# noamzilo/sed-crnn

Hardware: AMD Instinct MI355X
Metric: mel-frames/sec training throughput (seq=256, mel=40) (higher is better)
Workload: dtype f32; 1 GPU; BASELINE config 2: mono (B=128,256,40,1) per GPU, 3xConv3x3(128)+BN+ReLU+pool(1,2)+dropout0.5, BiGRU 2x128, Linear(256,1), BCEWithLogits, Adam lr 1e-3; full fit step (fwd+loss+bwd+allreduce+Adam); global_batch=128, seq_len=256, n_mels=40, parallelism=single

## Files before the change

### sed_crnn_amd/build.py

```python
import os
import subprocess
import sys
from concurrent.futures import ThreadPoolExecutor

HERE = os.path.dirname(os.path.abspath(__file__))
CSRC = os.path.join(HERE, "csrc")
OBJ = os.path.join(CSRC, "_obj")
LIB = os.path.join(HERE, "libsedcrnn.so")
SOURCES = ["api.cpp", "conv.hip", "conv_bf16.hip", "wino.hip", "conv1.hip", "bnpool.hip", "gemm.hip", "gru.hip", "misc.hip", "logmel.hip", "gcc.hip", "tdoa.hip", "doa.hip", "pcen.hip", "resample.hip", "data.hip", "detect.hip", "tune.hip", "stream.hip", "net.hip"]
FLAGS = ["--offload-arch=gfx950", "-O3", "-fPIC", "-std=c++17", "-Wall", "-Wno-unused-function"]
EXTRA_FLAGS = {"logmel.hip": ["-fno-slp-vectorize", "-Rpass-analysis=kernel-resource-usage"],
               "gcc.hip": ["-fno-slp-vectorize", "-Rpass-analysis=kernel-resource-usage"],
               "tdoa.hip": ["-fno-slp-vectorize", "-Rpass-analysis=kernel-resource-usage"],
               "doa.hip": ["-fno-slp-vectorize", "-Rpass-analysis=kernel-resource-usage"],
               "pcen.hip": ["-Rpass-analysis=kernel-resource-usage"],
               "conv.hip": ["-Rpass-analysis=kernel-resource-usage"],
               "wino.hip": ["-Rpass-analysis=kernel-resource-usage"],
               "conv_bf16.hip": ["-Rpass-analysis=kernel-resource-usage"]}
NO_SPILL_KERNELS = {"conv.hip": ("conv3x3_mfma_fwd2_k", "conv3x3_mfma_fwd_bf16x3_k")}
NO_SCRATCH_KERNELS = {"wino.hip": ("conv3x3_wino_k",),
                      "conv_bf16.hip": ("conv3x3_bf16_eval_k", "gemm_bf16_nt_k"),
                      "logmel.hip": ("logmel_fft_k",),
                      "gcc.hip": ("gcc_phat_k",),
                      "tdoa.hip": ("tdoa_accum_k", "tdoa_finish_k"),
                      "doa.hip": ("doa_steer_k",),
                      "pcen.hip": ("pcen_pass_k", "pcen_carry_k")}


def _hipcc():
    for c in (os.environ.get("HIPCC"), "/opt/rocm/bin/hipcc", "hipcc"):
        if c and (os.path.isabs(c) and os.path.exists(c) or not os.path.isabs(c)):
            return c
    raise RuntimeError("hipcc not found")


def _stale(target, deps):
    if not os.path.exists(target):
        return True
    t = os.path.getmtime(target)
    return any(os.path.getmtime(d) > t for d in deps)


def check_no_spill(remarks, kernels, allow_agprs=False):
    import re
    bad, seen, cur = [], set(), None
    for line in remarks.splitlines():
        m = re.search(r"remark: Function Name: (\S+)", line)
        if m:
            cur = next((k for k in kernels if k in m.group(1)), None)
            if cur:
                seen.add(cur)
            continue
        if cur:
            m = re.search(r"remark:\s+(ScratchSize \[bytes/lane\]|SGPRs Spill|VGPRs Spill|AGPRs): (\d+)", line)
            if m and int(m.group(2)) != 0 and not m.group(1).startswith("SGPRs") and not (allow_agprs and m.group(1) == "AGPRs"):
                bad.append(f"{cur}: {m.group(1)} = {m.group(2)}")
    bad += [f"{k}: no resource-usage remark found (kernel renamed? update NO_SPILL_KERNELS)" for k in kernels if k not in seen]
    return bad


def build(force=False, verbose=False):
    os.makedirs(OBJ, exist_ok=True)
    hipcc = _hipcc()
    headers = [os.path.join(CSRC, "common.h"), os.path.join(CSRC, "conv_shared.h"), os.path.join(CSRC, "detect_shared.h"), os.path.join(CSRC, "fft2048.h"), os.path.join(CSRC, "tdoa_shared.h"), os.path.join(HERE, "..", "include", "sedcrnn.h")]
    jobs = []
    objs = []
    for src in SOURCES:
        sp = os.path.join(CSRC, src)
        op = os.path.join(OBJ, os.path.splitext(src)[0] + ".o")
        objs.append(op)
        if force or _stale(op, [sp] + headers):
            cmd = [hipcc] + FLAGS + EXTRA_FLAGS.get(src, []) + (["-x", "hip"] if src.endswith(".cpp") else []) + ["-c", sp, "-o", op]
            jobs.append(cmd)

    def run(cmd):
        if verbose:
            print(" ".join(cmd), flush=True)
        r = subprocess.run(cmd, capture_output=True, text=True)
        if r.returncode != 0:
            raise RuntimeError("hipcc failed:\n" + " ".join(cmd) + "\n" + r.stdout + r.stderr)
        src = next((a for a in cmd if a.endswith((".hip", ".cpp"))), "")
        guarded = NO_SPILL_KERNELS.get(os.path.basename(src)) or NO_SCRATCH_KERNELS.get(os.path.basename(src))
        if guarded:
            bad = check_no_spill(r.stderr, guarded, allow_agprs=os.path.basename(src) in NO_SCRATCH_KERNELS)
            if bad:
                os.remove(cmd[cmd.index("-o") + 1])
                raise RuntimeError("hand-counted-waitcnt kernels must not spill:\n" + "\n".join(bad))
            keep, skip = [], 0
            for line in r.stderr.splitlines():
                if "remark:" in line:
                    skip = 2
                    continue
                if skip and (line.strip().startswith(("|", "^")) or " | " in line[:12]):
                    skip -= 1
                    continue
                skip = 0
                keep.append(line)
            return "\n".join(l for l in keep if l.strip() and "remarks generated" not in l)
        return r.stderr

    with ThreadPoolExecutor(max_workers=4) as ex:
        for warn in ex.map(run, jobs):
            if verbose and warn:
                print(warn)
    if force or jobs or _stale(LIB, objs):
        run([hipcc, "--offload-arch=gfx950", "-shared", "-fPIC", "-o", LIB] + objs)
    return LIB


if __name__ == "__main__":
    print(build(force="--force" in sys.argv, verbose=True))
```

### sed_crnn_amd/csrc/gru.hip

```cpp
#include "common.h"

static inline int gru_bt(int H, int B) {
    int bt = B >= 512 ? 4 : (B >= 256 ? 2 : 1);
    if (H >= 128 && bt > 2) bt = 2;
    return bt;
}

__global__ void gru_pack_whh_t_k(const float* __restrict__ w0, const float* __restrict__ w1,
                                 float* __restrict__ wt, int H) {
    int i = blockIdx.x * blockDim.x + threadIdx.x;
    int n = 3 * H * H;
    if (i >= 2 * n) return;
    int dir = i / n, e = i - dir * n;
    int g = e / H, k = e - g * H;
    const float* w = dir ? w1 : w0;
    wt[(size_t)dir * n + (size_t)k * 3 * H + g] = w[e];
}

constexpr int gru_nt(int hreg) { return hreg > 0 ? ((3 * hreg + 63) / 64) * 64 : 1024; }

__device__ __forceinline__ float gru_dot4(float w0, float w1, float w2, float w3, const f32x4& h) {
    return fmaf(w3, h[3], fmaf(w2, h[2], fmaf(w0, h[0], w1 * h[1])));
}

template <int HREG, int GRU_BT, int HTOT = HREG, int HLDS = 0>
__global__ __launch_bounds__(gru_nt(HTOT)) void gru_seq_fwd_k(
    const float* __restrict__ gi, const float* __restrict__ wt, const float* __restrict__ bhh0,
    const float* __restrict__ bhh1, float* __restrict__ out, float* __restrict__ saved, int B, int T, int H) {
    extern __shared__ __attribute__((aligned(16))) float smem[];
    float* h_s = smem;
    float* gh_s = smem + GRU_BT * H;
    float* w_l = smem + GRU_BT * 4 * H;
    const int g = threadIdx.x;
    const int dir = blockIdx.y, b0 = blockIdx.x * GRU_BT;
    const int H3 = 3 * H;
    const float* wtd = wt + (size_t)dir * H3 * H;
    const float* bhh = dir ? bhh1 : bhh0;
    const bool row = g < H3;
    const bool gate = g < H;
    constexpr bool HYB = HTOT != HREG && HREG > 0;

    float wreg[HREG > 0 ? HREG : 1];
    if (HREG > 0 && row) {
#pragma unroll
        for (int k = 0; k < HREG; ++k) wreg[k] = wtd[(size_t)k * H3 + g];
    }
    if (HYB && row) {
        for (int j = 0; j < HLDS; ++j) w_l[j * H3 + g] = wtd[(size_t)(HREG + j) * H3 + g];
    }
    const float bias = row ? bhh[g] : 0.f;
    for (int i = g; i < GRU_BT * H; i += blockDim.x) h_s[i] = 0.f;
    __syncthreads();

    float gr[GRU_BT], gz[GRU_BT], gn[GRU_BT], nr[GRU_BT], nz[GRU_BT], nn[GRU_BT], mr[GRU_BT], mz[GRU_BT], mn[GRU_BT];
    auto fetch_gi = [&](int s, float* a, float* bq, float* c) {
        const int tt = dir ? (T - 1 - s) : s;
#pragma unroll
        for (int b = 0; b < GRU_BT; ++b) {
            int bg = b0 + b;
            if (gate && bg < B && s < T) {
                const float* p = gi + (((size_t)bg * T + tt) * 2 + dir) * H3;
                a[b] = p[g]; bq[b] = p[H + g]; c[b] = p[2 * H + g];
            } else { a[b] = bq[b] = c[b] = 0.f; }
        }
    };
    fetch_gi(0, gr, gz, gn);
    fetch_gi(1, nr, nz, nn);
    for (int s = 0; s < T; ++s) {
        const int tt = dir ? (T - 1 - s) : s;
        fetch_gi(s + 2, mr, mz, mn);
        if (row) {
            float acc[GRU_BT];
#pragma unroll
            for (int b = 0; b < GRU_BT; ++b) acc[b] = bias;
            if (HREG > 0) {
#pragma unroll
                for (int k = 0; k < HREG; k += 4) {
#pragma unroll
                    for (int b = 0; b < GRU_BT; ++b) {
                        f32x4 hv = *(const f32x4*)(h_s + b * H + k);
                        acc[b] += gru_dot4(wreg[k], wreg[k + 1], wreg[k + 2], wreg[k + 3], hv);
                    }
                }
            }
            if (HYB) {
#pragma unroll 4
                for (int j = 0; j < HLDS; j += 4) {
                    const float w0 = w_l[j * H3 + g], w1 = w_l[(j + 1) * H3 + g], w2 = w_l[(j + 2) * H3 + g], w3 = w_l[(j + 3) * H3 + g];
#pragma unroll
                    for (int b = 0; b < GRU_BT; ++b) {
                        f32x4 hv = *(const f32x4*)(h_s + b * H + HREG + j);
                        acc[b] += gru_dot4(w0, w1, w2, w3, hv);
                    }
                }
            }
            if (HREG == 0 || HYB) {
                for (int k = HYB ? HREG + HLDS : 0; k < H; k += 4) {
                    float w0 = wtd[(size_t)k * H3 + g], w1 = wtd[(size_t)(k + 1) * H3 + g];
                    float w2 = wtd[(size_t)(k + 2) * H3 + g], w3 = wtd[(size_t)(k + 3) * H3 + g];
#pragma unroll
                    for (int b = 0; b < GRU_BT; ++b) {
                        f32x4 hv = *(const f32x4*)(h_s + b * H + k);
                        acc[b] += gru_dot4(w0, w1, w2, w3, hv);
                    }
                }
            }
#pragma unroll
            for (int b = 0; b < GRU_BT; ++b) gh_s[b * H3 + g] = acc[b];
        }
        __syncthreads();
        if (gate) {
#pragma unroll
            for (int b = 0; b < GRU_BT; ++b) {
                int bg = b0 + b;
                float ghr = gh_s[b * H3 + g], ghz = gh_s[b * H3 + H + g], ghn = gh_s[b * H3 + 2 * H + g];
                float hp = h_s[b * H + g];
                float r = __fdividef(1.f, 1.f + __expf(-(gr[b] + ghr)));
                float z = __fdividef(1.f, 1.f + __expf(-(gz[b] + ghz)));
                float a = gn[b] + r * ghn;
                float e2 = __expf(-2.f * fabsf(a));
                float n = copysignf(__fdividef(1.f - e2, 1.f + e2), a);
                float hn = (1.f - z) * n + z * hp;
                h_s[b * H + g] = hn;
                if (bg < B) {
                    out[((size_t)bg * T + tt) * 2 * H + dir * H + g] = hn;
                    if (saved) {
                        float* sp = saved + ((((size_t)bg * T + tt) * 2 + dir) * 5) * H + g;
                        sp[0] = r; sp[H] = z; sp[2 * H] = n; sp[3 * H] = ghn; sp[4 * H] = hp;
                    }
                }
            }
        }
#pragma unroll
        for (int b = 0; b < GRU_BT; ++b) {
            gr[b] = nr[b]; gz[b] = nz[b]; gn[b] = nn[b];
            nr[b] = mr[b]; nz[b] = mz[b]; nn[b] = mn[b];
        }
        __syncthreads();
    }
}

template <int HREG, int GRU_BT, int HTOT = HREG, int HLDS = 0>
__global__ __launch_bounds__(gru_nt(HTOT)) void gru_seq_bwd_k(
    const float* __restrict__ dout, const float* __restrict__ saved, const float* __restrict__ whh0,
    const float* __restrict__ whh1, float* __restrict__ dgi, float* __restrict__ dgh, float* __restrict__ bpart,
    int B, int T, int H) {
    extern __shared__ __attribute__((aligned(16))) float smem[];
    const int H3 = 3 * H;
    float* dgh_s = smem;
    float* part_s = smem + GRU_BT * H3;
    float* w_l = smem + GRU_BT * 2 * H3;
    const int g = threadIdx.x;
    const int dir = blockIdx.y, b0 = blockIdx.x * GRU_BT;
    const float* whh = dir ? whh1 : whh0;
    const bool row = g < H3;
    const bool gate = g < H;
    const int p = g / H, k = g - p * H;
    constexpr bool HYB = HTOT != HREG && HREG > 0;

    float wreg[HREG > 0 ? HREG : 1];
    if (HREG > 0 && row) {
#pragma unroll
        for (int j = 0; j < HREG; ++j) wreg[j] = whh[((size_t)p * H + j) * H + k];
    }
    if (HYB && row) {
        for (int j = 0; j < HLDS; ++j) w_l[j * H3 + g] = whh[((size_t)p * H + HREG + j) * H + k];
    }
    for (int i = g; i < 3 * GRU_BT * H; i += blockDim.x) part_s[i] = 0.f;
    float dhc[GRU_BT];
#pragma unroll
    for (int b = 0; b < GRU_BT; ++b) dhc[b] = 0.f;
    float sb0 = 0.f, sb1 = 0.f, sb2 = 0.f, sb3 = 0.f;
    __syncthreads();

    float cs[GRU_BT][6], ns[GRU_BT][6], ms[GRU_BT][6];
    auto fetch_sv = [&](int s, float (*q)[6]) {
        const int tt = dir ? s : (T - 1 - s);
#pragma unroll
        for (int b = 0; b < GRU_BT; ++b) {
            int bg = b0 + b;
            if (gate && bg < B && s < T) {
                const float* sp = saved + ((((size_t)bg * T + tt) * 2 + dir) * 5) * H + g;
                q[b][0] = sp[0]; q[b][1] = sp[H]; q[b][2] = sp[2 * H]; q[b][3] = sp[3 * H]; q[b][4] = sp[4 * H];
                q[b][5] = dout[((size_t)bg * T + tt) * 2 * H + dir * H + g];
            }
        }
    };
    constexpr bool AHEAD2 = !(HREG == 0 && GRU_BT == 4) && !HYB;
    fetch_sv(0, cs);
    if (AHEAD2) fetch_sv(1, ns);
    for (int s = 0; s < T; ++s) {
        const int tt = dir ? s : (T - 1 - s);
        if (AHEAD2) fetch_sv(s + 2, ms);
        else fetch_sv(s + 1, ns);
        if (gate) {
#pragma unroll
            for (int b = 0; b < GRU_BT; ++b) {
                int bg = b0 + b;
                float dr_pre = 0.f, dz_pre = 0.f, dn_pre = 0.f, dghn = 0.f, carry = 0.f;
                if (bg < B) {
                    float r = cs[b][0], z = cs[b][1], n = cs[b][2], ghn = cs[b][3], hp = cs[b][4];
                    float dh = cs[b][5] + dhc[b] +
                               part_s[(0 * GRU_BT + b) * H + g] + part_s[(1 * GRU_BT + b) * H + g] +
                               part_s[(2 * GRU_BT + b) * H + g];
                    float dn = dh * (1.f - z);
                    float dz = dh * (hp - n);
                    carry = dh * z;
                    dn_pre = dn * (1.f - n * n);
                    dz_pre = dz * z * (1.f - z);
                    float dr = dn_pre * ghn;
                    dghn = dn_pre * r;
                    dr_pre = dr * r * (1.f - r);
                    size_t o = (((size_t)bg * T + tt) * 2 + dir) * H3 + g;
                    dgi[o] = dr_pre; dgi[o + H] = dz_pre; dgi[o + 2 * H] = dn_pre;
                    dgh[o] = dr_pre; dgh[o + H] = dz_pre; dgh[o + 2 * H] = dghn;
                }
                dhc[b] = carry;
                sb0 += dr_pre; sb1 += dz_pre; sb2 += dn_pre; sb3 += dghn;
                dgh_s[b * H3 + g] = dr_pre; dgh_s[b * H3 + H + g] = dz_pre; dgh_s[b * H3 + 2 * H + g] = dghn;
            }
        }
        __syncthreads();
        if (row) {
            float acc[GRU_BT];
#pragma unroll
            for (int b = 0; b < GRU_BT; ++b) acc[b] = 0.f;
            if (HREG > 0) {
#pragma unroll
                for (int j = 0; j < HREG; j += 4) {
#pragma unroll
                    for (int b = 0; b < GRU_BT; ++b) {
                        f32x4 dv = *(const f32x4*)(dgh_s + b * H3 + p * H + j);
                        acc[b] += wreg[j] * dv[0] + wreg[j + 1] * dv[1] + wreg[j + 2] * dv[2] + wreg[j + 3] * dv[3];
                    }
                }
            }
            if (HYB) {
#pragma unroll 4
                for (int j = 0; j < HLDS; j += 4) {
                    const float w0 = w_l[j * H3 + g], w1 = w_l[(j + 1) * H3 + g], w2 = w_l[(j + 2) * H3 + g], w3 = w_l[(j + 3) * H3 + g];
#pragma unroll
                    for (int b = 0; b < GRU_BT; ++b) {
                        f32x4 dv = *(const f32x4*)(dgh_s + b * H3 + p * H + HREG + j);
                        acc[b] += w0 * dv[0] + w1 * dv[1] + w2 * dv[2] + w3 * dv[3];
                    }
                }
            }
            if (HREG == 0 || HYB) {
                for (int j = HYB ? HREG + HLDS : 0; j < H; j += 4) {
                    const float* wp = whh + ((size_t)p * H + j) * H + k;
                    float w0 = wp[0], w1 = wp[H], w2 = wp[2 * H], w3 = wp[3 * H];
#pragma unroll
                    for (int b = 0; b < GRU_BT; ++b) {
                        f32x4 dv = *(const f32x4*)(dgh_s + b * H3 + p * H + j);
                        acc[b] += w0 * dv[0] + w1 * dv[1] + w2 * dv[2] + w3 * dv[3];
                    }
                }
            }
#pragma unroll
            for (int b = 0; b < GRU_BT; ++b) part_s[(p * GRU_BT + b) * H + k] = acc[b];
        }
#pragma unroll
        for (int b = 0; b < GRU_BT; ++b)
#pragma unroll
            for (int e = 0; e < 6; ++e) { cs[b][e] = ns[b][e]; if (AHEAD2) ns[b][e] = ms[b][e]; }
        __syncthreads();
    }
    if (bpart && gate) {
        float* bp = bpart + ((size_t)(blockIdx.x * 2 + dir) * 4) * H + g;
        bp[0] = sb0; bp[H] = sb1; bp[2 * H] = sb2; bp[3 * H] = sb3;
    }
}

__global__ void gru_bias_grad_k(const float* __restrict__ bpart, int nblk, int H, float* __restrict__ dbih0,
                                float* __restrict__ dbih1, float* __restrict__ dbhh0, float* __restrict__ dbhh1) {
    int i = blockIdx.x * blockDim.x + threadIdx.x;
    if (i >= 2 * 4 * H) return;
    int j = i % H, c = (i / H) % 4, dir = i / (4 * H);
    float a = 0.f;
#pragma unroll 8
    for (int b = 0; b < nblk; ++b) a += bpart[((size_t)(b * 2 + dir) * 4 + c) * H + j];
    float* dbih = dir ? dbih1 : dbih0;
    float* dbhh = dir ? dbhh1 : dbhh0;
    if (c < 3) dbih[c * H + j] = a;
    if (c < 2) dbhh[c * H + j] = a;
    if (c == 3) dbhh[2 * H + j] = a;
}

static int gru_threads(int H) { return ((3 * H + 63) / 64) * 64; }
#define GRU_HR 96
#define GRU_HL 48
#define GRU_HR_FWD 116

extern "C" size_t sed_gru_seq_workspace_bytes(int H) { return (size_t)2 * 3 * H * H * sizeof(float); }

struct GruVariant { int bt, hreg, hlds; };
static inline GruVariant gru_variant(int H, int B, int hyb_hreg) {
    const int bt = gru_bt(H, B);
    if (H == 8 || H == 16 || H == 32 || H == 64 || H == 128) return {bt, H, 0};
    if (H == 256 && bt == 1) return {bt, hyb_hreg, GRU_HL};
    return {bt, 0, 0};
}

extern "C" int sed_gru_seq_variant(int B, int H, int* bt, int* hreg, int* hlds) {
    SED_REQUIRE(bt && hreg && hlds, "gru_seq_variant: null pointer");
    SED_REQUIRE(B > 0 && H > 0 && H % 4 == 0 && 3 * H <= 1024, "gru_seq_variant: H=%d must be a multiple of 4 and <= 341", H);
    const GruVariant v = gru_variant(H, B, GRU_HR_FWD);
    *bt = v.bt; *hreg = v.hreg; *hlds = v.hlds;
    return 0;
}

#define GRU_BT3(HR, KERNEL, ...)                                                              \
    if (v.bt == 1) KERNEL<HR, 1><<<grid, nt, lds, s>>>(__VA_ARGS__);                          \
    else if (v.bt == 2) KERNEL<HR, 2><<<grid, nt, lds, s>>>(__VA_ARGS__);                     \
    else KERNEL<HR, 4><<<grid, nt, lds, s>>>(__VA_ARGS__)
#define GRU_DISPATCH(KERNEL, ...)                                                             \
    if (v.hlds > 0) {                                                                         \
        KERNEL<GRU_HRX, 1, 256, GRU_HL><<<grid, nt, lds + (size_t)GRU_HL * 768 * sizeof(float), s>>>(__VA_ARGS__); \
    } else switch (v.hreg) {                                                                  \
        case 8: GRU_BT3(8, KERNEL, __VA_ARGS__); break;                                       \
        case 16: GRU_BT3(16, KERNEL, __VA_ARGS__); break;                                     \
        case 32: GRU_BT3(32, KERNEL, __VA_ARGS__); break;                                     \
        case 64: GRU_BT3(64, KERNEL, __VA_ARGS__); break;                                     \
        case 128:                                                                             \
            if (v.bt == 1) KERNEL<128, 1><<<grid, nt, lds, s>>>(__VA_ARGS__);                 \
            else KERNEL<128, 2><<<grid, nt, lds, s>>>(__VA_ARGS__);                           \
            break;                                                                            \
        default: GRU_BT3(0, KERNEL, __VA_ARGS__); break;                                      \
    }

extern "C" int sed_gru_seq_fwd(const float* gi, const float* const* whh, const float* const* bhh, float* out,
                               float* saved, void* workspace, int B, int T, int H, void* stream) {
    SED_REQUIRE(gi && whh && bhh && out && workspace && whh[0] && whh[1] && bhh[0] && bhh[1], "gru_seq_fwd: null pointer");
    SED_REQUIRE(B > 0 && T > 0 && H > 0 && H % 4 == 0 && 3 * H <= 1024, "gru_seq_fwd: H=%d must be a multiple of 4 and <= 341", H);
    hipStream_t s = as_stream(stream);
    float* wt = (float*)workspace;
    int n = 2 * 3 * H * H;
    gru_pack_whh_t_k<<<cdiv(n, 256), 256, 0, s>>>(whh[0], whh[1], wt, H);
    SED_LAUNCH_CHECK("gru_pack_whh_t");
    const GruVariant v = gru_variant(H, B, GRU_HR_FWD);
    dim3 grid(cdiv(B, v.bt), 2);
    int nt = gru_threads(H);
    size_t lds = (size_t)v.bt * 4 * H * sizeof(float);
    SedProfScope prof(SED_K_GRU_FWD, s, 2.0 * 2 * B * (double)T * 3 * H * H);
    if (v.hlds > 0)
        (void)hipFuncSetAttribute((const void*)gru_seq_fwd_k<GRU_HR_FWD, 1, 256, GRU_HL>, hipFuncAttributeMaxDynamicSharedMemorySize, 160 * 1024);
#define GRU_HRX GRU_HR_FWD
    GRU_DISPATCH(gru_seq_fwd_k, gi, wt, bhh[0], bhh[1], out, saved, B, T, H);
#undef GRU_HRX
    SED_LAUNCH_CHECK("gru_seq_fwd");
    return 0;
}

extern "C" size_t sed_gru_seq_bwd_workspace_bytes(int B, int H) { return (size_t)cdiv(B, gru_bt(H, B)) * 2 * 4 * H * sizeof(float); }

extern "C" int sed_gru_seq_bwd(const float* dout, const float* saved, const float* const* whh, float* dgi,
                               float* dgh, float* const* dbih, float* const* dbhh, void* workspace, int B, int T,
                               int H, void* stream) {
    SED_REQUIRE(dout && saved && whh && whh[0] && whh[1] && dgi && dgh, "gru_seq_bwd: null pointer");
    const bool want_bias = dbih && dbhh;
    SED_REQUIRE(!want_bias || (workspace && dbih[0] && dbih[1] && dbhh[0] && dbhh[1]), "gru_seq_bwd: bias gradients need all four outputs and a workspace");
    float* bpart = want_bias ? (float*)workspace : nullptr;
    SED_REQUIRE(B > 0 && T > 0 && H > 0 && H % 4 == 0 && 3 * H <= 1024, "gru_seq_bwd: H=%d must be a multiple of 4 and <= 341", H);
    hipStream_t s = as_stream(stream);
    const GruVariant v = gru_variant(H, B, GRU_HR);
    dim3 grid(cdiv(B, v.bt), 2);
    int nt = gru_threads(H);
    size_t lds = (size_t)v.bt * 6 * H * sizeof(float);
    SedProfScope prof(SED_K_GRU_BWD, s, 2.0 * 2 * B * (double)T * 3 * H * H);
    if (v.hlds > 0)
        (void)hipFuncSetAttribute((const void*)gru_seq_bwd_k<GRU_HR, 1, 256, GRU_HL>, hipFuncAttributeMaxDynamicSharedMemorySize, 160 * 1024);
#define GRU_HRX GRU_HR
    GRU_DISPATCH(gru_seq_bwd_k, dout, saved, whh[0], whh[1], dgi, dgh, bpart, B, T, H);
#undef GRU_HRX
    SED_LAUNCH_CHECK("gru_seq_bwd");
    if (want_bias) {
        gru_bias_grad_k<<<cdiv(8 * H, 256), 256, 0, s>>>(bpart, cdiv(B, v.bt), H, dbih[0], dbih[1], dbhh[0], dbhh[1]);
        SED_LAUNCH_CHECK("gru_bias_grad");
    }
    return 0;
}
```

Measured before the change: 5.902 million mel-frames/s.

## Software-pipeline GRU recurrence with inline-asm loads and hand-counted vmcnt waits

Rewrites the forward and backward GRU sequence kernels to use a rotating three-slot prefetch buffer. Per-step gate inputs and saved activations are fetched with inline-asm global loads, and the code waits on explicit vmcnt counts instead of letting the compiler insert full waits. The register matvec is split into batched LDS loads with sched barriers, and the step loop is unrolled by three so buffer indices are compile-time constants. The build now guards these kernels against spills, because the hand-counted waits and register pinning break if the compiler spills. Out-of-range batch and time indices are clamped instead of masked.

```diff
diff --git a/sed_crnn_amd/build.py b/sed_crnn_amd/build.py
--- a/sed_crnn_amd/build.py
+++ b/sed_crnn_amd/build.py
@@ -16,8 +16,10 @@
                "pcen.hip": ["-Rpass-analysis=kernel-resource-usage"],
                "conv.hip": ["-Rpass-analysis=kernel-resource-usage"],
                "wino.hip": ["-Rpass-analysis=kernel-resource-usage"],
-               "conv_bf16.hip": ["-Rpass-analysis=kernel-resource-usage"]}
-NO_SPILL_KERNELS = {"conv.hip": ("conv3x3_mfma_fwd2_k", "conv3x3_mfma_fwd_bf16x3_k")}
+               "conv_bf16.hip": ["-Rpass-analysis=kernel-resource-usage"],
+               "gru.hip": ["-Rpass-analysis=kernel-resource-usage"]}
+NO_SPILL_KERNELS = {"conv.hip": ("conv3x3_mfma_fwd2_k", "conv3x3_mfma_fwd_bf16x3_k"),
+                    "gru.hip": ("gru_seq_fwd_k", "gru_seq_bwd_k")}
 NO_SCRATCH_KERNELS = {"wino.hip": ("conv3x3_wino_k",),
                       "conv_bf16.hip": ("conv3x3_bf16_eval_k", "gemm_bf16_nt_k"),
                       "logmel.hip": ("logmel_fft_k",),
diff --git a/sed_crnn_amd/csrc/gru.hip b/sed_crnn_amd/csrc/gru.hip
--- a/sed_crnn_amd/csrc/gru.hip
+++ b/sed_crnn_amd/csrc/gru.hip
@@ -21,6 +21,46 @@
 
 __device__ __forceinline__ float gru_dot4(float w0, float w1, float w2, float w3, const f32x4& h) {
     return fmaf(w3, h[3], fmaf(w2, h[2], fmaf(w0, h[0], w1 * h[1])));
+}
+
+template <int N> __device__ __forceinline__ void gru_vmcnt() {
+    static_assert(N >= 0 && N <= 63, "vmcnt is a 6-bit field on gfx9");
+    asm volatile("s_waitcnt vmcnt(%0)" ::"n"(N) : "memory");
+}
+__device__ __forceinline__ void gru_load(float& dst, unsigned voff, const float* sbase) {
+    asm volatile("global_load_dword %0, %1, %2" : "=&v"(dst) : "v"(voff), "s"(sbase) : "memory");
+}
+template <int V> struct GruC { static constexpr int value = V; };
+
+template <int HREG, int BT, int LB>
+__device__ __forceinline__ void gru_dot_reg(const float (&w)[HREG > 0 ? HREG : 1], const float* x, int stride, float (&acc)[BT]) {
+    constexpr int NQ = HREG / 4 * BT, NB = (NQ + LB - 1) / LB;
+    f32x4 v[2][LB];
+#pragma unroll
+    for (int j = 0; j < LB; ++j)
+        if (j < NQ) v[0][j] = *(const f32x4*)(x + (j % BT) * stride + (j / BT) * 4);
+    __builtin_amdgcn_sched_barrier(0);
+#pragma unroll
+    for (int nb = 0; nb < NB; ++nb) {
+#pragma unroll
+        for (int j = 0; j < LB; ++j) {
+            const int i = (nb + 1) * LB + j;
+            if (i < NQ) v[(nb + 1) & 1][j] = *(const f32x4*)(x + (i % BT) * stride + (i / BT) * 4);
+        }
+        const int last = (nb + 1) * LB <= NQ ? LB - 1 : NQ - nb * LB - 1;
+        __builtin_amdgcn_sched_barrier(0);
+        asm volatile("" : "+v"(v[nb & 1][last]));
+        __builtin_amdgcn_sched_barrier(0);
+#pragma unroll
+        for (int j = 0; j < LB; ++j) {
+            const int i = nb * LB + j;
+            if (i < NQ) {
+                const int k = (i / BT) * 4;
+                acc[i % BT] += gru_dot4(w[k], w[k + 1], w[k + 2], w[k + 3], v[nb & 1][j]);
+            }
+        }
+        __builtin_amdgcn_sched_barrier(0);
+    }
 }
 
 template <int HREG, int GRU_BT, int HTOT = HREG, int HLDS = 0>
@@ -39,6 +79,7 @@
     const bool row = g < H3;
     const bool gate = g < H;
     constexpr bool HYB = HTOT != HREG && HREG > 0;
+    constexpr bool ROT = !HYB;
 
     float wreg[HREG > 0 ? HREG : 1];
     if (HREG > 0 && row) {
@@ -52,28 +93,13 @@
     for (int i = g; i < GRU_BT * H; i += blockDim.x) h_s[i] = 0.f;
     __syncthreads();
 
-    float gr[GRU_BT], gz[GRU_BT], gn[GRU_BT], nr[GRU_BT], nz[GRU_BT], nn[GRU_BT], mr[GRU_BT], mz[GRU_BT], mn[GRU_BT];
-    auto fetch_gi = [&](int s, float* a, float* bq, float* c) {
-        const int tt = dir ? (T - 1 - s) : s;
-#pragma unroll
-        for (int b = 0; b < GRU_BT; ++b) {
-            int bg = b0 + b;
-            if (gate && bg < B && s < T) {
-                const float* p = gi + (((size_t)bg * T + tt) * 2 + dir) * H3;
-                a[b] = p[g]; bq[b] = p[H + g]; c[b] = p[2 * H + g];
-            } else { a[b] = bq[b] = c[b] = 0.f; }
-        }
-    };
-    fetch_gi(0, gr, gz, gn);
-    fetch_gi(1, nr, nz, nn);
-    for (int s = 0; s < T; ++s) {
-        const int tt = dir ? (T - 1 - s) : s;
-        fetch_gi(s + 2, mr, mz, mn);
+    auto matvec = [&](float b_hh) __attribute__((always_inline)) {
         if (row) {
             float acc[GRU_BT];
 #pragma unroll
-            for (int b = 0; b < GRU_BT; ++b) acc[b] = bias;
-            if (HREG > 0) {
+            for (int b = 0; b < GRU_BT; ++b) acc[b] = b_hh;
+            if (HREG > 0 && ROT) gru_dot_reg<HREG, GRU_BT, 8>(wreg, h_s, H, acc);
+            if (HREG > 0 && !ROT) {
 #pragma unroll
                 for (int k = 0; k < HREG; k += 4) {
 #pragma unroll
@@ -108,35 +134,112 @@
 #pragma unroll
             for (int b = 0; b < GRU_BT; ++b) gh_s[b * H3 + g] = acc[b];
         }
-        __syncthreads();
+    };
+    auto gates = [&](int tt, const float (&q)[GRU_BT][3], bool sv) __attribute__((always_inline)) {
         if (gate) {
 #pragma unroll
             for (int b = 0; b < GRU_BT; ++b) {
                 int bg = b0 + b;
                 float ghr = gh_s[b * H3 + g], ghz = gh_s[b * H3 + H + g], ghn = gh_s[b * H3 + 2 * H + g];
                 float hp = h_s[b * H + g];
-                float r = __fdividef(1.f, 1.f + __expf(-(gr[b] + ghr)));
-                float z = __fdividef(1.f, 1.f + __expf(-(gz[b] + ghz)));
-                float a = gn[b] + r * ghn;
+                float r = __fdividef(1.f, 1.f + __expf(-(q[b][0] + ghr)));
+                float z = __fdividef(1.f, 1.f + __expf(-(q[b][1] + ghz)));
+                float a = q[b][2] + r * ghn;
                 float e2 = __expf(-2.f * fabsf(a));
                 float n = copysignf(__fdividef(1.f - e2, 1.f + e2), a);
                 float hn = (1.f - z) * n + z * hp;
                 h_s[b * H + g] = hn;
-                if (bg < B) {
+                if (GRU_BT == 1 || bg < B) {
                     out[((size_t)bg * T + tt) * 2 * H + dir * H + g] = hn;
-                    if (saved) {
+                    if (sv) {
                         float* sp = saved + ((((size_t)bg * T + tt) * 2 + dir) * 5) * H + g;
                         sp[0] = r; sp[H] = z; sp[2 * H] = n; sp[3 * H] = ghn; sp[4 * H] = hp;
                     }
                 }
             }
         }
-#pragma unroll
-        for (int b = 0; b < GRU_BT; ++b) {
-            gr[b] = nr[b]; gz[b] = nz[b]; gn[b] = nn[b];
-            nr[b] = mr[b]; nz[b] = mz[b]; nn[b] = mn[b];
-        }
-        __syncthreads();
+    };
+
+    constexpr int AHEAD = 2, NSET = AHEAD + 1;
+    float pf[NSET][GRU_BT][3];
+    if constexpr (ROT) {
+        const int gq = g % H;
+        const unsigned vo0 = 4u * gq, vo1 = 4u * (H + gq), vo2 = 4u * (2 * H + gq);
+        auto fetch_gi = [&](int s, float (&q)[GRU_BT][3]) __attribute__((always_inline)) {
+            const int sc = s < T ? s : T - 1;
+            const int tt = dir ? (T - 1 - sc) : sc;
+#pragma unroll
+            for (int b = 0; b < GRU_BT; ++b) {
+                const int bg = b0 + b < B ? b0 + b : B - 1;
+                const float* p = gi + (((size_t)bg * T + tt) * 2 + dir) * H3;
+                gru_load(q[b][0], vo0, p); gru_load(q[b][1], vo1, p); gru_load(q[b][2], vo2, p);
+            }
+        };
+        fetch_gi(0, pf[0]);
+        fetch_gi(1, pf[1]);
+        gru_vmcnt<0>();
+        if (HREG > 0) {
+#pragma unroll
+            for (int k = 0; k < HREG; ++k) asm volatile("" : "+v"(wreg[k]));
+        }
+        float bias_r = bias;
+        asm volatile("" : "+v"(bias_r));
+
+        auto step = [&](int s, auto RC, auto SV) __attribute__((always_inline)) {
+            constexpr int R = decltype(RC)::value;
+            constexpr bool SAVED = decltype(SV)::value != 0;
+            constexpr int NWAIT = AHEAD * 3 * GRU_BT + (GRU_BT == 1 ? AHEAD * (SAVED ? 6 : 1) : 0);
+            fetch_gi(s + AHEAD, pf[(R + AHEAD) % NSET]);
+            matvec(bias_r);
+            __syncthreads();
+            gru_vmcnt<NWAIT>();
+#pragma unroll
+            for (int b = 0; b < GRU_BT; ++b)
+#pragma unroll
+                for (int e = 0; e < 3; ++e) asm volatile("" : "+v"(pf[R][b][e]));
+            gates(dir ? (T - 1 - s) : s, pf[R], SAVED);
+            __syncthreads();
+        };
+        auto run = [&](auto SV) __attribute__((always_inline)) {
+            int s = 0;
+            for (; s + NSET <= T; s += NSET) { step(s, GruC<0>{}, SV); step(s + 1, GruC<1>{}, SV); step(s + 2, GruC<2>{}, SV); }
+            if (s < T) step(s, GruC<0>{}, SV);
+            if (s + 1 < T) step(s + 1, GruC<1>{}, SV);
+        };
+        if (saved) run(GruC<1>{});
+        else run(GruC<0>{});
+        gru_vmcnt<0>();
+#pragma unroll
+        for (int r = 0; r < NSET; ++r)
+#pragma unroll
+            for (int b = 0; b < GRU_BT; ++b)
+#pragma unroll
+                for (int e = 0; e < 3; ++e) asm volatile("" : "+v"(pf[r][b][e]));
+    } else {
+        auto fetch_gi = [&](int s, float (&q)[GRU_BT][3]) __attribute__((always_inline)) {
+            const int tt = dir ? (T - 1 - s) : s;
+#pragma unroll
+            for (int b = 0; b < GRU_BT; ++b) {
+                int bg = b0 + b;
+                if (gate && bg < B && s < T) {
+                    const float* p = gi + (((size_t)bg * T + tt) * 2 + dir) * H3;
+                    q[b][0] = p[g]; q[b][1] = p[H + g]; q[b][2] = p[2 * H + g];
+                } else { q[b][0] = q[b][1] = q[b][2] = 0.f; }
+            }
+        };
+        fetch_gi(0, pf[0]);
+        fetch_gi(1, pf[1]);
+        for (int s = 0; s < T; ++s) {
+            fetch_gi(s + 2, pf[2]);
+            matvec(bias);
+            __syncthreads();
+            gates(dir ? (T - 1 - s) : s, pf[0], saved != nullptr);
+#pragma unroll
+            for (int b = 0; b < GRU_BT; ++b)
+#pragma unroll
+                for (int e = 0; e < 3; ++e) { pf[0][b][e] = pf[1][b][e]; pf[1][b][e] = pf[2][b][e]; }
+            __syncthreads();
+        }
     }
 }
 
@@ -157,6 +260,7 @@
     const bool gate = g < H;
     const int p = g / H, k = g - p * H;
     constexpr bool HYB = HTOT != HREG && HREG > 0;
+    constexpr bool ROT = HREG == HTOT && HREG > 0 && HREG * GRU_BT < 256;
 
     float wreg[HREG > 0 ? HREG : 1];
     if (HREG > 0 && row) {
@@ -173,32 +277,13 @@
     float sb0 = 0.f, sb1 = 0.f, sb2 = 0.f, sb3 = 0.f;
     __syncthreads();
 
-    float cs[GRU_BT][6], ns[GRU_BT][6], ms[GRU_BT][6];
-    auto fetch_sv = [&](int s, float (*q)[6]) {
-        const int tt = dir ? s : (T - 1 - s);
-#pragma unroll
-        for (int b = 0; b < GRU_BT; ++b) {
-            int bg = b0 + b;
-            if (gate && bg < B && s < T) {
-                const float* sp = saved + ((((size_t)bg * T + tt) * 2 + dir) * 5) * H + g;
-                q[b][0] = sp[0]; q[b][1] = sp[H]; q[b][2] = sp[2 * H]; q[b][3] = sp[3 * H]; q[b][4] = sp[4 * H];
-                q[b][5] = dout[((size_t)bg * T + tt) * 2 * H + dir * H + g];
-            }
-        }
-    };
-    constexpr bool AHEAD2 = !(HREG == 0 && GRU_BT == 4) && !HYB;
-    fetch_sv(0, cs);
-    if (AHEAD2) fetch_sv(1, ns);
-    for (int s = 0; s < T; ++s) {
-        const int tt = dir ? s : (T - 1 - s);
-        if (AHEAD2) fetch_sv(s + 2, ms);
-        else fetch_sv(s + 1, ns);
+    auto gates = [&](int tt, const float (&cs)[GRU_BT][6]) __attribute__((always_inline)) {
         if (gate) {
 #pragma unroll
             for (int b = 0; b < GRU_BT; ++b) {
                 int bg = b0 + b;
                 float dr_pre = 0.f, dz_pre = 0.f, dn_pre = 0.f, dghn = 0.f, carry = 0.f;
-                if (bg < B) {
+                if (GRU_BT == 1 || bg < B) {
                     float r = cs[b][0], z = cs[b][1], n = cs[b][2], ghn = cs[b][3], hp = cs[b][4];
                     float dh = cs[b][5] + dhc[b] +
                                part_s[(0 * GRU_BT + b) * H + g] + part_s[(1 * GRU_BT + b) * H + g] +
@@ -216,55 +301,165 @@
                     dgh[o] = dr_pre; dgh[o + H] = dz_pre; dgh[o + 2 * H] = dghn;
                 }
                 dhc[b] = carry;
+                asm volatile("" : "+v"(dr_pre), "+v"(dz_pre), "+v"(dn_pre), "+v"(dghn));
                 sb0 += dr_pre; sb1 += dz_pre; sb2 += dn_pre; sb3 += dghn;
                 dgh_s[b * H3 + g] = dr_pre; dgh_s[b * H3 + H + g] = dz_pre; dgh_s[b * H3 + 2 * H + g] = dghn;
             }
         }
-        __syncthreads();
+    };
+    auto matvec = [&]() __attribute__((always_inline)) {
         if (row) {
             float acc[GRU_BT];
 #pragma unroll
             for (int b = 0; b < GRU_BT; ++b) acc[b] = 0.f;
-            if (HREG > 0) {
-#pragma unroll
-                for (int j = 0; j < HREG; j += 4) {
-#pragma unroll
-                    for (int b = 0; b < GRU_BT; ++b) {
-                        f32x4 dv = *(const f32x4*)(dgh_s + b * H3 + p * H + j);
-                        acc[b] += wreg[j] * dv[0] + wreg[j + 1] * dv[1] + wreg[j + 2] * dv[2] + wreg[j + 3] * dv[3];
-                    }
-                }
-            }
-            if (HYB) {
+            gru_dot_reg<HREG, GRU_BT, 8>(wreg, dgh_s + p * H, H3, acc);
+#pragma unroll
+            for (int b = 0; b < GRU_BT; ++b) part_s[(p * GRU_BT + b) * H + k] = acc[b];
+        }
+    };
+
+    if constexpr (ROT) {
+        constexpr int AHEAD = 2, NSET = AHEAD + 1;
+        float sv[NSET][GRU_BT][6];
+        const unsigned vo = 4u * (g % H);
+        auto fetch_sv = [&](int s, float (&q)[GRU_BT][6]) __attribute__((always_inline)) {
+            const int sc = s < T ? s : T - 1;
+            const int tt = dir ? sc : (T - 1 - sc);
+#pragma unroll
+            for (int b = 0; b < GRU_BT; ++b) {
+                const int bg = b0 + b < B ? b0 + b : B - 1;
+                const float* sp = saved + ((((size_t)bg * T + tt) * 2 + dir) * 5) * H;
+#pragma unroll
+                for (int e = 0; e < 5; ++e) gru_load(q[b][e], vo, sp + (size_t)e * H);
+                gru_load(q[b][5], vo, dout + ((size_t)bg * T + tt) * 2 * H + dir * H);
+            }
+        };
+        fetch_sv(0, sv[0]);
+        fetch_sv(1, sv[1]);
+        gru_vmcnt<0>();
+        if (HREG > 0) {
+#pragma unroll
+            for (int j = 0; j < HREG; ++j) asm volatile("" : "+v"(wreg[j]));
+        }
+        auto step = [&](int s, auto RC) __attribute__((always_inline)) {
+            constexpr int R = decltype(RC)::value;
+            constexpr int NWAIT = AHEAD * 6 * GRU_BT + (GRU_BT == 1 ? AHEAD * 6 : 0);
+            fetch_sv(s + AHEAD, sv[(R + AHEAD) % NSET]);
+            gru_vmcnt<NWAIT>();
+#pragma unroll
+            for (int b = 0; b < GRU_BT; ++b)
+#pragma unroll
+                for (int e = 0; e < 6; ++e) asm volatile("" : "+v"(sv[R][b][e]));
+            gates(dir ? s : (T - 1 - s), sv[R]);
+            __syncthreads();
+            matvec();
+            __syncthreads();
+        };
+        int s = 0;
+        for (; s + NSET <= T; s += NSET) { step(s, GruC<0>{}); step(s + 1, GruC<1>{}); step(s + 2, GruC<2>{}); }
+        if (s < T) step(s, GruC<0>{});
+        if (s + 1 < T) step(s + 1, GruC<1>{});
+        gru_vmcnt<0>();
+#pragma unroll
+        for (int r = 0; r < NSET; ++r)
+#pragma unroll
+            for (int b = 0; b < GRU_BT; ++b)
+#pragma unroll
+                for (int e = 0; e < 6; ++e) asm volatile("" : "+v"(sv[r][b][e]));
+    } else {
+        float cs[GRU_BT][6], ns[GRU_BT][6], ms[GRU_BT][6];
+        auto fetch_sv = [&](int s, float (*q)[6]) {
+            const int tt = dir ? s : (T - 1 - s);
+#pragma unroll
+            for (int b = 0; b < GRU_BT; ++b) {
+                int bg = b0 + b;
+                if (gate && bg < B && s < T) {
+                    const float* sp = saved + ((((size_t)bg * T + tt) * 2 + dir) * 5) * H + g;
+                    q[b][0] = sp[0]; q[b][1] = sp[H]; q[b][2] = sp[2 * H]; q[b][3] = sp[3 * H]; q[b][4] = sp[4 * H];
+                    q[b][5] = dout[((size_t)bg * T + tt) * 2 * H + dir * H + g];
+                }
+            }
+        };
+        constexpr bool AHEAD2 = !(HREG == 0 && GRU_BT == 4) && !HYB;
+        fetch_sv(0, cs);
+        if (AHEAD2) fetch_sv(1, ns);
+        for (int s = 0; s < T; ++s) {
+            const int tt = dir ? s : (T - 1 - s);
+            if (AHEAD2) fetch_sv(s + 2, ms);
+            else fetch_sv(s + 1, ns);
+            if (gate) {
+#pragma unroll
+                for (int b = 0; b < GRU_BT; ++b) {
+                    int bg = b0 + b;
+                    float dr_pre = 0.f, dz_pre = 0.f, dn_pre = 0.f, dghn = 0.f, carry = 0.f;
+                    if (bg < B) {
+                        float r = cs[b][0], z = cs[b][1], n = cs[b][2], ghn = cs[b][3], hp = cs[b][4];
+                        float dh = cs[b][5] + dhc[b] +
+                                   part_s[(0 * GRU_BT + b) * H + g] + part_s[(1 * GRU_BT + b) * H + g] +
+                                   part_s[(2 * GRU_BT + b) * H + g];
+                        float dn = dh * (1.f - z);
+                        float dz = dh * (hp - n);
+                        carry = dh * z;
+                        dn_pre = dn * (1.f - n * n);
+                        dz_pre = dz * z * (1.f - z);
+                        float dr = dn_pre * ghn;
+                        dghn = dn_pre * r;
+                        dr_pre = dr * r * (1.f - r);
+                        size_t o = (((size_t)bg * T + tt) * 2 + dir) * H3 + g;
+                        dgi[o] = dr_pre; dgi[o + H] = dz_pre; dgi[o + 2 * H] = dn_pre;
+                        dgh[o] = dr_pre; dgh[o + H] = dz_pre; dgh[o + 2 * H] = dghn;
+                    }
+                    dhc[b] = carry;
+                    sb0 += dr_pre; sb1 += dz_pre; sb2 += dn_pre; sb3 += dghn;
+                    dgh_s[b * H3 + g] = dr_pre; dgh_s[b * H3 + H + g] = dz_pre; dgh_s[b * H3 + 2 * H + g] = dghn;
+                }
+            }
+            __syncthreads();
+            if (row) {
+                float acc[GRU_BT];
+#pragma unroll
+                for (int b = 0; b < GRU_BT; ++b) acc[b] = 0.f;
+                if (HREG > 0) {
+#pragma unroll
+                    for (int j = 0; j < HREG; j += 4) {
+#pragma unroll
+                        for (int b = 0; b < GRU_BT; ++b) {
+                            f32x4 dv = *(const f32x4*)(dgh_s + b * H3 + p * H + j);
+                            acc[b] += wreg[j] * dv[0] + wreg[j + 1] * dv[1] + wreg[j + 2] * dv[2] + wreg[j + 3] * dv[3];
+                        }
+                    }
+                }
+                if (HYB) {
 #pragma unroll 4
-                for (int j = 0; j < HLDS; j += 4) {
-                    const float w0 = w_l[j * H3 + g], w1 = w_l[(j + 1) * H3 + g], w2 = w_l[(j + 2) * H3 + g], w3 = w_l[(j + 3) * H3 + g];
-#pragma unroll
-                    for (int b = 0; b < GRU_BT; ++b) {
-                        f32x4 dv = *(const f32x4*)(dgh_s + b * H3 + p * H + HREG + j);
-                        acc[b] += w0 * dv[0] + w1 * dv[1] + w2 * dv[2] + w3 * dv[3];
-                    }
-                }
-            }
-            if (HREG == 0 || HYB) {
-                for (int j = HYB ? HREG + HLDS : 0; j < H; j += 4) {
-                    const float* wp = whh + ((size_t)p * H + j) * H + k;
-                    float w0 = wp[0], w1 = wp[H], w2 = wp[2 * H], w3 = wp[3 * H];
-#pragma unroll
-                    for (int b = 0; b < GRU_BT; ++b) {
-                        f32x4 dv = *(const f32x4*)(dgh_s + b * H3 + p * H + j);
-                        acc[b] += w0 * dv[0] + w1 * dv[1] + w2 * dv[2] + w3 * dv[3];
-                    }
-                }
-            }
-#pragma unroll
-            for (int b = 0; b < GRU_BT; ++b) part_s[(p * GRU_BT + b) * H + k] = acc[b];
-        }
-#pragma unroll
-        for (int b = 0; b < GRU_BT; ++b)
-#pragma unroll
-            for (int e = 0; e < 6; ++e) { cs[b][e] = ns[b][e]; if (AHEAD2) ns[b][e] = ms[b][e]; }
-        __syncthreads();
+                    for (int j = 0; j < HLDS; j += 4) {
+                        const float w0 = w_l[j * H3 + g], w1 = w_l[(j + 1) * H3 + g], w2 = w_l[(j + 2) * H3 + g], w3 = w_l[(j + 3) * H3 + g];
+#pragma unroll
+                        for (int b = 0; b < GRU_BT; ++b) {
+                            f32x4 dv = *(const f32x4*)(dgh_s + b * H3 + p * H + HREG + j);
+                            acc[b] += w0 * dv[0] + w1 * dv[1] + w2 * dv[2] + w3 * dv[3];
+                        }
+                    }
+                }
+                if (HREG == 0 || HYB) {
+                    for (int j = HYB ? HREG + HLDS : 0; j < H; j += 4) {
+                        const float* wp = whh + ((size_t)p * H + j) * H + k;
+                        float w0 = wp[0], w1 = wp[H], w2 = wp[2 * H], w3 = wp[3 * H];
+#pragma unroll
+                        for (int b = 0; b < GRU_BT; ++b) {
+                            f32x4 dv = *(const f32x4*)(dgh_s + b * H3 + p * H + j);
+                            acc[b] += w0 * dv[0] + w1 * dv[1] + w2 * dv[2] + w3 * dv[3];
+                        }
+                    }
+                }
+#pragma unroll
+                for (int b = 0; b < GRU_BT; ++b) part_s[(p * GRU_BT + b) * H + k] = acc[b];
+            }
+#pragma unroll
+            for (int b = 0; b < GRU_BT; ++b)
+#pragma unroll
+                for (int e = 0; e < 6; ++e) { cs[b][e] = ns[b][e]; if (AHEAD2) ns[b][e] = ms[b][e]; }
+            __syncthreads();
+        }
     }
     if (bpart && gate) {
         float* bp = bpart + ((size_t)(blockIdx.x * 2 + dir) * 4) * H + g;
```

Measured after the change: 5.905 million mel-frames/s (median of 3 runs). Within noise of the previous version (+0.0%).
